# FrancescoI/torchrecsys

Measured on AMD Instinct MI355X. Metric: training interactions/sec (pos+neg), higher is better.
Workload: dtype f32; 1 GPU; c4 per-GPU shard: net_type='fm', 10M users x 1M items, 125M-interaction shard of 1B, dim=128, per-GPU batch 32768 (global 262144 at 8 GPUs); global_batch=32768, per_gpu_batch=32768, rng=device (Feistel epoch shuffle + Philox4x32-10 negative sampler)

## Files before the change

### torchrecsys_amd/csrc/api.cpp

```cpp
#include "trs_common.h"

#include <string.h>

static thread_local char g_err[512] = "";

void trs_set_error(const char* fmt, ...) {
  va_list ap;
  va_start(ap, fmt);
  vsnprintf(g_err, sizeof(g_err), fmt, ap);
  va_end(ap);
}

extern "C" const char* trs_last_error(void) { return g_err; }

#include <mutex>
#include <stdlib.h>

namespace {
struct Knob {
  const char* name;
  int64_t TrsTuning::*wide;
  int TrsTuning::*narrow;
  int64_t unset;
};
const Knob KNOBS[] = {
    {"GRID_CAP", &TrsTuning::grid_cap, nullptr, 256 * 16},
    {"PASS_GRID_CAP", &TrsTuning::pass_grid_cap, nullptr, 4096},
    {"PRESORT_GRID_CAP", &TrsTuning::presort_grid_cap, nullptr, 512},
    {"K1_ITERS", nullptr, &TrsTuning::k1_iters, 0},
    {"PASS_ITERS", nullptr, &TrsTuning::pass_iters, 0},
    {"PASS_NT", nullptr, &TrsTuning::pass_nt, -1},
    {"K1_NT", nullptr, &TrsTuning::k1_nt, -1},
    {"K1_WGS_PER_CU", nullptr, &TrsTuning::k1_wgs_per_cu, 2},
    {"K1_APPLY_IN_LOOP", nullptr, &TrsTuning::k1_apply_in_loop, 1},
    {"K1_APPLY_STATS", nullptr, &TrsTuning::k1_apply_stats, 0},
    {"GEMM32_NO_GLDS", nullptr, &TrsTuning::gemm32_no_glds, 0},
    {"GEMM16_TN_WIDE", nullptr, &TrsTuning::gemm16_tn_wide, -1},
    {"GEMM16_TILE", nullptr, &TrsTuning::gemm16_tile, 0},
    {"GEMM16_NO_GLDS", nullptr, &TrsTuning::gemm16_no_glds, 0},
    {"BN_FINAL_TWO_SWEEPS", nullptr, &TrsTuning::bn_final_two_sweeps, 0},
    {"FOLDIN_DEPTH", nullptr, &TrsTuning::foldin_depth, 4},
    {"RANKS_STAGES", nullptr, &TrsTuning::ranks_stages, 3},
    {"EASE_STAGES", nullptr, &TrsTuning::ease_stages, 7},
};
TrsTuning g_tuning;
std::once_flag g_tuning_once;
void knob_store(const Knob& k, int64_t v) {
  if (k.wide) g_tuning.*(k.wide) = v;
  else g_tuning.*(k.narrow) = (int)v;
}
}

TrsTuning& trs_tuning() {
  std::call_once(g_tuning_once, [] {
    for (const Knob& k : KNOBS) {
      char name[64];
      snprintf(name, sizeof(name), "TRS_%s", k.name);
      const char* e = getenv(name);
      knob_store(k, (e && *e) ? atoll(e) : k.unset);
    }
  });
  return g_tuning;
}

extern "C" int trs_tuning_set(const char* name, int64_t value, int32_t unset) {
  TRS_REQUIRE(name != nullptr, "trs_tuning_set: NULL name");
  (void)trs_tuning();
  for (const Knob& k : KNOBS)
    if (strcmp(k.name, name) == 0) {
      knob_store(k, unset ? k.unset : value);
      return TRS_OK;
    }
  trs_set_error("trs_tuning_set: unknown knob %s", name);
  return TRS_E_ARG;
}

extern "C" int trs_abi_version(void) { return TRS_ABI_VERSION; }

extern "C" int trs_check_device(void) {
  int dev = -1;
  if (hipGetDevice(&dev) != hipSuccess) {
    trs_set_error("trs_check_device: no HIP device");
    (void)hipGetLastError();
    return TRS_E_DEVICE;
  }
  hipDeviceProp_t p;
  if (hipGetDeviceProperties(&p, dev) != hipSuccess) {
    trs_set_error("trs_check_device: hipGetDeviceProperties failed");
    (void)hipGetLastError();
    return TRS_E_DEVICE;
  }
  if (strncmp(p.gcnArchName, "gfx950", 6) != 0) {
    trs_set_error("trs_check_device: device %d is %s, this library is built for gfx950 only", dev, p.gcnArchName);
    return TRS_E_DEVICE;
  }
  return TRS_OK;
}

extern "C" int trs_events_create(int32_t n, void** handles_out) {
  TRS_REQUIRE(n >= 0 && (n == 0 || handles_out), "trs_events_create: bad arguments");
  for (int32_t i = 0; i < n; ++i) {
    hipEvent_t e;
    if (hipEventCreate(&e) != hipSuccess) {
      trs_set_error("trs_events_create: hipEventCreate failed");
      (void)hipGetLastError();
      return TRS_E_LAUNCH;
    }
    handles_out[i] = (void*)e;
  }
  return TRS_OK;
}

extern "C" int trs_events_destroy(int32_t n, void** handles) {
  for (int32_t i = 0; i < n; ++i)
    if (handles && handles[i]) (void)hipEventDestroy((hipEvent_t)handles[i]);
  return TRS_OK;
}

// ... 10 lines not shown
```

### torchrecsys_amd/csrc/fast_step.hip

```cpp
#include "score_kernels.h"
#include "opt_rows.h"

#include <math.h>
#include <stdlib.h>

namespace trs {

struct FastArgs {
  trs_tables T;
  int32_t* user;
  int32_t* pos;
  int32_t* neg;
  int64_t B;
  int32_t* err;
  int from_stream;
  const int2* sui;
  const int32_t* neg_static;
  int64_t N;
  uint64_t shuffle_key;
  int hb;
  int64_t t0;
  uint64_t sample_seed;
  uint64_t sample_offset;
  float* gz;
  float* du;
  float inv_B;
  float lr;
  int loss;
  float* loss_sum;
  uint64_t* uown;
  uint64_t* iown;
  uint32_t* udup;
  uint32_t* idup;
  uint32_t stamp;
  const uint8_t* udup_pos;
  const uint8_t* idup_pos;
  float* ustage;
  OptArgs o;
  uint32_t* sync;
  uint32_t sync_base, sync_target;
  const int32_t* nflag;
  int apply_in_loop, apply_stats;
};

struct RawIds {
  int32_t u, p, n;
  uint8_t dup;
  uint16_t idup;
  int64_t v;
  bool valid;
};

struct TripleIds {
  int32_t u, p, n;
  bool valid, ok, dup, pdup, ndup;
};

template <int SRC, int INL>
__device__ __forceinline__ RawIds issue_ids(const FastArgs& a, int64_t t) {
  RawIds r;
  r.valid = t < a.B;
  const int64_t tc = r.valid ? t : a.B - 1;
  r.v = 0;
  if (SRC != 0) {
    const int64_t p = trs_feistel_perm(a.t0 + tc, a.N, a.shuffle_key, a.hb);
    const int2 ui = a.sui[p];
    r.u = ui.x;
    r.p = ui.y;
    if (SRC == 2) {
      r.n = a.neg_static[p];
    } else {
      const trs_u4 x = trs_philox4x32_10(a.sample_offset + (uint64_t)tc, a.sample_seed);
      const uint64_t x64 = ((uint64_t)x.y << 32) | (uint64_t)x.x;
      r.v = a.T.n_items > 1 ? (int64_t)trs_mulhi64(x64, (uint64_t)(a.T.n_items - 1)) : 0;
      r.n = 0;
    }
  } else {
    r.u = a.user[tc];
    r.p = a.pos[tc];
    r.n = a.neg[tc];
  }
  r.dup = 1;
  r.idup = 0x0101;
  if (INL) r.dup = a.udup_pos[tc];
  if (INL >= 2) r.idup = reinterpret_cast<const uint16_t*>(a.idup_pos)[tc];
  return r;
}

template <int SRC>
__device__ __forceinline__ TripleIds finalize_ids(const FastArgs& a, const RawIds& w) {
  TripleIds r;
  r.valid = w.valid;
  int64_t uid = w.u, pid = w.p;
  int64_t nid = SRC == 1 ? (a.T.n_items > 1 ? w.v + (w.v >= pid ? 1 : 0) : 0) : (int64_t)w.n;
  r.ok = true;
  if ((uint64_t)uid >= (uint64_t)a.T.n_users) { r.ok = false; uid = 0; }
  if ((uint64_t)pid >= (uint64_t)a.T.n_items) { r.ok = false; pid = 0; }
  if ((uint64_t)nid >= (uint64_t)a.T.n_items) { r.ok = false; nid = 0; }
  r.u = (int32_t)uid;
  r.p = (int32_t)pid;
  r.n = (int32_t)nid;
  r.dup = w.dup != 0;
  r.pdup = (w.idup & 0x00ffu) != 0;
  r.ndup = (w.idup & 0xff00u) != 0;
  return r;
}

template <int VEC, int K>
struct TripleRows {
  RowReg<VEC, K> u, pi, ni;
  float ul, pl, nl;
  RowReg<VEC, K> us1, us2;
  float uls1, uls2;
};

template <int VEC, int G, int K, bool FULL, int OPT, int NTU = 0>
__device__ __forceinline__ void load_rows(TripleRows<VEC, K>& r, const trs_tables& T, const OptArgs& o,
                                          const TripleIds& id, int lig) {
  row_load<VEC, G, K, FULL, (NTU & 1) != 0>(r.u, T.user, id.u, T.D, lig);
  row_load<VEC, G, K, FULL>(r.pi, T.item, id.p, T.D, lig);
  row_load<VEC, G, K, FULL>(r.ni, T.item, id.n, T.D, lig);
  r.ul = T.user_lin[id.u];
  r.pl = T.item_lin[id.p];
  r.nl = T.item_lin[id.n];
  if (OPT != OPT_SGD) {
    row_load<VEC, G, K, FULL>(r.us1, o.user_s1, id.u, T.D, lig);
    r.uls1 = o.user_lin_s1[id.u];
    if (OPT == OPT_ADAM) {
      row_load<VEC, G, K, FULL>(r.us2, o.user_s2, id.u, T.D, lig);
      r.uls2 = o.user_lin_s2[id.u];
    }
  }
}

constexpr int DEFER_ITERS = 8;
struct DeferEntry {
  uint32_t tw;
  int32_t row;
  float c;
  float clin;
};

template <int NET, int VEC, int G, int K, int SRC, bool FULL, int INL, int OPT = OPT_SGD, int NTU = 0>
__global__ __launch_bounds__(TRS_BLOCK, (INL == 3 && VEC == 4 && G >= 4 && K == 1 && FULL) ? 4 : 1) void fwd_stage_kernel(const FastArgs a) {
  constexpr int N = K * VEC;
  constexpr int TPW = TRS_WAVE / G;
  constexpr bool DEFER = INL == 3;
  constexpr int NWV = TRS_BLOCK / TRS_WAVE;
  constexpr int LIST_CAP = DEFER ? NWV * DEFER_ITERS * TPW * 3 : 1;
  __shared__ DeferEntry s_list[LIST_CAP];
  __shared__ int s_total;
  const trs_tables& T = a.T;
  const int D = T.D;
  const int64_t B = a.B;
  const int lane = threadIdx.x & 63;
  const int lig = lane % G;
  const int64_t wave = ((int64_t)blockIdx.x * TRS_BLOCK + threadIdx.x) >> 6;
  const int64_t nwave = ((int64_t)gridDim.x * TRS_BLOCK) >> 6;
  const int64_t stride = nwave * TPW;
  float loss_acc = 0.f;

#ifdef TRS_K1_STAMPS
  uint64_t* stamps = reinterpret_cast<uint64_t*>(a.gz) + 8 * (int64_t)blockIdx.x;
  if (INL == 3 && threadIdx.x == 0) {
    stamps[0] = __builtin_amdgcn_s_memrealtime();
    stamps[4] = 0;
  }
#endif
  __shared__ int s_arr;
  __shared__ int s_left;
  int64_t fi = 0;
  bool early = false, arrived = false;
  if (DEFER) {
    if (threadIdx.x == 0) s_total = s_arr = s_left = 0;
    if (a.nflag) {
      const int64_t nf = *a.nflag;
      fi = (nf + stride - 1) / stride;
      early = fi < (B + stride - 1) / stride;
    }
    __syncthreads();
  }
  auto arrive = [&]() {
    int before = 0;
    if (lane == 0) before = atomicAdd(&s_arr, 1);
    before = __builtin_amdgcn_readfirstlane(before);
    if (before == NWV - 1 && lane == 0)
      (void)__hip_atomic_fetch_add(a.sync, 1u, __ATOMIC_RELAXED, __HIP_MEMORY_SCOPE_AGENT);
    arrived = true;
  };
  constexpr int CAPW = DEFER_ITERS * TPW * 3, DU = 4, KDD = (N * G + TRS_WAVE - 1) / TRS_WAVE;
  const int wv = __builtin_amdgcn_readfirstlane((int)(threadIdx.x >> 6));
  int my_cnt = 0, next_e = 0;
  bool complete = false;
  auto entry_at = [&](int e) -> int { return early ? wv * CAPW + e : wv + NWV * e; };
  auto load_round = [&](float (&x)[DU][KDD], int e0, int n_mine) {
#pragma unroll
    for (int k = 0; k < DU; ++k) {
      const bool has = e0 + k < n_mine;
      const DeferEntry en = s_list[has ? entry_at(e0 + k) : 0];
      const int64_t tk = has ? (int64_t)(en.tw >> 2) : 0;
      const float* src = ((en.tw & 3u) == 0 ? a.du : a.ustage) + tk * (int64_t)D;
#pragma unroll
      for (int q = 0; q < KDD; ++q) {
        const int e = q * TRS_WAVE + lane;
        x[k][q] = __hip_atomic_load(src + (e < D ? e : 0), __ATOMIC_RELAXED, __HIP_MEMORY_SCOPE_AGENT);
      }
    }
  };
  auto apply_round = [&](float (&x)[DU][KDD], int e0, int n_mine) {
#pragma unroll
    for (int k = 0; k < DU; ++k) {
      if (e0 + k >= n_mine) continue;
      const DeferEntry en = s_list[entry_at(e0 + k)];
      const int which = (int)(en.tw & 3u);
      float* dst = (which == 0 ? T.user : T.item) + (int64_t)en.row * D;
#pragma unroll
      for (int q = 0; q < KDD; ++q) {
        const int e = q * TRS_WAVE + lane;
        if (e < D) atomicAdd(dst + e, en.c * x[k][q]);
      }
      if (lane == 0) atomicAdd((which == 0 ? T.user_lin : T.item_lin) + en.row, en.clin);
    }
  };
  int64_t t = wave * TPW + lane / G;
// ... 1018 lines not shown
static int launch_meta_stage_mt(const ScoreArgs& a, hipStream_t s) {
  RowCfg c;
  TRS_TRY(row_cfg_for("launch_meta_stage", a.T.D, c));
  const int tpw = TRS_WAVE / c.g;
  int64_t iters = (a.Bt.B + 512 * 4 * (int64_t)tpw - 1) / (512 * 4 * (int64_t)tpw);
  iters = iters < 2 ? 2 : (iters > 8 ? 8 : iters);
  int64_t grid = ((a.Bt.B + tpw - 1) / tpw + 4 * iters - 1) / (4 * iters);
  grid = grid < 1 ? 1 : (grid > 4096 ? 4096 : grid);
  const dim3 gr((unsigned)grid), bl(TRS_BLOCK);
  return for_whole_row_shape(c, [&](auto V, auto G, auto K) {
    const bool full = V() * G() * K() == a.T.D;
    if (a.o.kind != OPT_SGD) {
      if (!full) return 1;
      if (a.o.kind == OPT_ADAM)
        hipLaunchKernelGGL((meta_stage_kernel<NET, V(), G(), K(), true, MT, OPT_ADAM>), gr, bl, 0, s, a);
      else
        hipLaunchKernelGGL((meta_stage_kernel<NET, V(), G(), K(), true, MT, OPT_ADAGRAD>), gr, bl, 0, s, a);
    } else if (full)
      hipLaunchKernelGGL((meta_stage_kernel<NET, V(), G(), K(), true, MT>), gr, bl, 0, s, a);
    else
      hipLaunchKernelGGL((meta_stage_kernel<NET, V(), G(), K(), false, MT>), gr, bl, 0, s, a);
    TRS_CHECK_LAUNCH("meta_stage_kernel");
    return TRS_OK;
  });
}

template <int NET>
static int launch_meta_stage(const ScoreArgs& a, hipStream_t s) {
  if (!a.Bt.pos_meta || !a.Bt.neg_meta || a.grad_rows) return 1;
  switch (a.T.M) {
    case 1: return launch_meta_stage_mt<NET, 1>(a, s);
    case 2: return launch_meta_stage_mt<NET, 2>(a, s);
    case 3: return launch_meta_stage_mt<NET, 3>(a, s);
    default: return 1;
  }
}

template <typename KernelT>
static int64_t defer_resident_cap(KernelT kernel) {
  int occ = 0, dev = 0, cus = 0;
  if (hipOccupancyMaxActiveBlocksPerMultiprocessor(&occ, kernel, TRS_BLOCK, 0) != hipSuccess) return 0;
  if (hipGetDevice(&dev) != hipSuccess ||
      hipDeviceGetAttribute(&cus, hipDeviceAttributeMultiprocessorCount, dev) != hipSuccess)
    return 0;
  const int want = trs_tuning().k1_wgs_per_cu;
  const int per_cu = occ - 1 < want ? occ - 1 : want;
  return per_cu > 0 ? (int64_t)per_cu * cus : 0;
}

enum StepForm { STEP_MARKS, STEP_SORTED_MARKS, STEP_SORTED, STEP_FLAGS };
struct StepPlan {
  StepForm form;
  int src;
  int inl;
  int item_bits;
  bool owners;
  bool adaptive;
  bool user_pairs;
  bool meta;
  bool meta_ids;
  bool meta_sorted;
  bool sync;
  bool nflag;
};

template <int NET>
static int launch_fwd_stage(const FastArgs& a, const StepPlan& p, hipStream_t s, uint32_t* deferred) {
  *deferred = 0;
  RowCfg c;
  TRS_TRY(row_cfg_for("launch_fwd_stage", a.T.D, c));
  const int tpw = TRS_WAVE / c.g;
  const int iters_env = trs_tuning().k1_iters;
  int64_t iters = iters_env > 0 ? iters_env : (a.B + 512 * 4 * (int64_t)tpw - 1) / (512 * 4 * (int64_t)tpw);
  if (iters < 2) iters = 2;
  if (iters > 8 && iters_env <= 0) iters = 8;
  int64_t grid = ((a.B + tpw - 1) / tpw + 4 * iters - 1) / (4 * iters);
  if (grid < 1) grid = 1;
  if (grid > 4096) grid = 4096;
  const int ntu_env = trs_tuning().k1_nt;
  const int ntu = ntu_env >= 0 ? ntu_env : ((int64_t)a.T.n_users * a.T.D * 4 > ((int64_t)512 << 20) ? 3 : 0);
  const dim3 gr((unsigned)grid), bl(TRS_BLOCK);
  return for_row_shape(c, [&](auto V, auto G, auto K) {
    constexpr int VV = V(), GG = G(), KK = K();
    auto launch = [&](auto FULL) {
      constexpr bool FU = FULL();
      if (p.inl == 1 && a.o.kind == OPT_ADAM)
        hipLaunchKernelGGL((fwd_stage_kernel<NET, VV, GG, KK, 0, FU, 1, OPT_ADAM>), gr, bl, 0, s, a);
      else if (p.inl == 1 && a.o.kind == OPT_ADAGRAD)
        hipLaunchKernelGGL((fwd_stage_kernel<NET, VV, GG, KK, 0, FU, 1, OPT_ADAGRAD>), gr, bl, 0, s, a);
      else if (p.inl == 1)
        hipLaunchKernelGGL((fwd_stage_kernel<NET, VV, GG, KK, 0, FU, 1>), gr, bl, 0, s, a);
      else if (p.inl == 3 && iters <= DEFER_ITERS) {
        static const int64_t cap = defer_resident_cap(fwd_stage_kernel<NET, VV, GG, KK, 0, FU, 3>);
        if (grid <= cap) {
          FastArgs b = a;
          b.sync_target = a.sync_base + (uint32_t)grid;
          b.apply_in_loop = trs_tuning().k1_apply_in_loop != 0;
          b.apply_stats = trs_tuning().k1_apply_stats != 0;
          if (ntu == 1)
            hipLaunchKernelGGL((fwd_stage_kernel<NET, VV, GG, KK, 0, FU, 3, OPT_SGD, 1>), gr, bl, 0, s, b);
          else if (ntu == 3)
            hipLaunchKernelGGL((fwd_stage_kernel<NET, VV, GG, KK, 0, FU, 3, OPT_SGD, 3>), gr, bl, 0, s, b);
          else
            hipLaunchKernelGGL((fwd_stage_kernel<NET, VV, GG, KK, 0, FU, 3>), gr, bl, 0, s, b);
          *deferred = (uint32_t)grid;
        } else
          hipLaunchKernelGGL((fwd_stage_kernel<NET, VV, GG, KK, 0, FU, 2>), gr, bl, 0, s, a);
      } else if (p.inl >= 2)
        hipLaunchKernelGGL((fwd_stage_kernel<NET, VV, GG, KK, 0, FU, 2>), gr, bl, 0, s, a);
      else if (p.src == 0) hipLaunchKernelGGL((fwd_stage_kernel<NET, VV, GG, KK, 0, FU, 0>), gr, bl, 0, s, a);
      else if (p.src == 1) hipLaunchKernelGGL((fwd_stage_kernel<NET, VV, GG, KK, 1, FU, 0>), gr, bl, 0, s, a);
      else hipLaunchKernelGGL((fwd_stage_kernel<NET, VV, GG, KK, 2, FU, 0>), gr, bl, 0, s, a);
    };
    if (VV * GG * KK == a.T.D) launch(std::true_type{});
    else launch(std::false_type{});
    TRS_CHECK_LAUNCH("fwd_stage_kernel");
    return TRS_OK;
  });
}

static int launch_flagged_update(const FastArgs& a, hipStream_t s) {
  const dim3 gr(trs_grid((3 * a.B + FLG_REFS - 1) / FLG_REFS, TRS_BLOCK / TRS_WAVE)), bl(TRS_BLOCK);
  const int kd = (a.T.D + TRS_WAVE - 1) / TRS_WAVE;
  if (kd <= 1) hipLaunchKernelGGL(flagged_update_kernel<1>, gr, bl, 0, s, a);
  else if (kd <= 2) hipLaunchKernelGGL(flagged_update_kernel<2>, gr, bl, 0, s, a);
  else if (kd <= 4) hipLaunchKernelGGL(flagged_update_kernel<4>, gr, bl, 0, s, a);
  else if (kd <= 8) hipLaunchKernelGGL(flagged_update_kernel<8>, gr, bl, 0, s, a);
  else hipLaunchKernelGGL(flagged_update_kernel<16>, gr, bl, 0, s, a);
  TRS_CHECK_LAUNCH("flagged_update_kernel");
  return TRS_OK;
}

template <int WHICH>
static int launch_plain(const FastArgs& a, hipStream_t s) {
  RowCfg c;
  TRS_TRY(row_cfg_for("launch_plain", a.T.D, c));
  const int per = (TRS_WAVE / c.g) * 2;
  const dim3 gr(trs_grid((a.B + per - 1) / per, TRS_BLOCK / TRS_WAVE)), bl(TRS_BLOCK);
  return for_row_shape(c, [&](auto V, auto G, auto K) {
    constexpr int VV = V(), GG = G(), KK = K();
    auto launch = [&](auto FULL) {
      if (WHICH == 0) hipLaunchKernelGGL((item_owner_update_kernel<VV, GG, KK, FULL()>), gr, bl, 0, s, a);
      else if (WHICH == 1) hipLaunchKernelGGL((user_plain_update_kernel<VV, GG, KK, FULL()>), gr, bl, 0, s, a);
      else hipLaunchKernelGGL((user_dup_update_kernel<VV, GG, KK, FULL()>), gr, bl, 0, s, a);
    };
    if (VV * GG * KK == a.T.D) launch(std::true_type{});
    else launch(std::false_type{});
    TRS_CHECK_LAUNCH("plain update kernel");
    return TRS_OK;
  });
}

static int launch_updates(const FastArgs& a, bool owners, hipStream_t s, hipEvent_t ev_k3) {
  const int D = a.T.D;
  if (owners) {
    int rc = launch_plain<0>(a, s);
    if (rc) return rc;
  }
#define TRS_UPD(L, KD, U)                                                                            \
  {                                                                                                  \
    constexpr int PER = (TRS_WAVE / L) * U;                                                          \
    const dim3 gr(trs_grid((a.B + PER - 1) / PER, TRS_BLOCK / TRS_WAVE)), bl(TRS_BLOCK);             \
    if (owners) {                                                                                    \
      hipLaunchKernelGGL((item_update_kernel<L, KD, U, 2>), gr, bl, 0, s, a);                        \
      if (ev_k3) (void)hipEventRecord(ev_k3, s);                                                     \
    } else {                                                                                         \
// ... 411 lines not shown
```

### torchrecsys_amd/csrc/trs_common.h

```cpp
#pragma once
#include <hip/hip_runtime.h>
#include <stdint.h>
#include <stdio.h>
#include <stdarg.h>
#include <stdlib.h>

#include "../../include/trs.h"

#define TRS_WAVE 64
#define TRS_BLOCK 256

void trs_set_error(const char* fmt, ...);

#define TRS_REQUIRE(cond, ...)        \
  do {                                \
    if (!(cond)) {                    \
      trs_set_error(__VA_ARGS__);     \
      return TRS_E_ARG;               \
    }                                 \
  } while (0)

#define TRS_TRY(expr)           \
  do {                          \
    const int rc__ = (expr);    \
    if (rc__) return rc__;      \
  } while (0)

#define TRS_CHECK_LAUNCH(name)                                           \
  do {                                                                     \
    hipError_t e__ = hipGetLastError();                                    \
    if (e__ != hipSuccess) {                                               \
      trs_set_error("%s: launch failed: %s", name, hipGetErrorString(e__)); \
      return TRS_E_LAUNCH;                                                 \
    }                                                                      \
  } while (0)

static inline double trs_as_written(float x) {
  char buf[40];
  for (int digits = 1; digits <= 9; ++digits) {
    snprintf(buf, sizeof buf, "%.*g", digits, (double)x);
    if (strtof(buf, nullptr) == x) return strtod(buf, nullptr);
  }
  return (double)x;
}

struct TrsTuning {
  int64_t grid_cap;
  int64_t pass_grid_cap;
  int64_t presort_grid_cap;
  int k1_iters;
  int pass_iters;
  int pass_nt;
  int k1_nt;
  int k1_wgs_per_cu;
  int k1_apply_in_loop;
  int k1_apply_stats;
  int gemm32_no_glds;
  int gemm16_tn_wide;
  int gemm16_tile;
  int gemm16_no_glds;
  int bn_final_two_sweeps;
  int foldin_depth;
  int ranks_stages;
  int ease_stages;
};
TrsTuning& trs_tuning();

static inline int trs_grid(int64_t work_items, int items_per_block) {
  const int64_t cap = trs_tuning().grid_cap;
  int64_t g = (work_items + items_per_block - 1) / items_per_block;
  if (g < 1) g = 1;
  if (g > cap) g = cap;
  return (int)g;
}

__device__ __forceinline__ int64_t trs_ld_idx(const void* p, int idx_bytes, int64_t t) {
  return idx_bytes == 8 ? ((const int64_t*)p)[t] : (int64_t)((const int32_t*)p)[t];
}
__device__ __forceinline__ void trs_st_idx(void* p, int idx_bytes, int64_t t, int64_t v) {
  if (idx_bytes == 8)
    ((int64_t*)p)[t] = v;
  else
    ((int32_t*)p)[t] = (int32_t)v;
}

struct trs_u4 {
  uint32_t x, y, z, w;
};
__host__ __device__ __forceinline__ trs_u4 trs_philox4x32_10(uint64_t counter, uint64_t key) {
  uint32_t c0 = (uint32_t)counter, c1 = (uint32_t)(counter >> 32), c2 = 0u, c3 = 0u;
  uint32_t k0 = (uint32_t)key, k1 = (uint32_t)(key >> 32);
#pragma unroll
  for (int r = 0; r < 10; ++r) {
    uint64_t p0 = (uint64_t)0xD2511F53u * c0;
    uint64_t p1 = (uint64_t)0xCD9E8D57u * c2;
    uint32_t n0 = (uint32_t)(p1 >> 32) ^ c1 ^ k0;
    uint32_t n1 = (uint32_t)p1;
    uint32_t n2 = (uint32_t)(p0 >> 32) ^ c3 ^ k1;
    uint32_t n3 = (uint32_t)p0;
    c0 = n0; c1 = n1; c2 = n2; c3 = n3;
    k0 += 0x9E3779B9u;
    k1 += 0xBB67AE85u;
  }
  trs_u4 o = {c0, c1, c2, c3};
  return o;
}

__host__ __device__ __forceinline__ uint64_t trs_mulhi64(uint64_t a, uint64_t b) {
#ifdef __HIP_DEVICE_COMPILE__
  return __umul64hi(a, b);
#else
  return (uint64_t)(((unsigned __int128)a * (unsigned __int128)b) >> 64);
#endif
}

__host__ __device__ __forceinline__ int64_t trs_sample_one_neg(uint64_t seed, uint64_t ctr, int64_t pos,
                                                               int64_t n_items) {
  trs_u4 r = trs_philox4x32_10(ctr, seed);
  uint64_t x = ((uint64_t)r.y << 32) | (uint64_t)r.x;
  if (n_items <= 1) return 0;
  int64_t v = (int64_t)trs_mulhi64(x, (uint64_t)(n_items - 1));
  return v + (v >= pos ? 1 : 0);
}

__device__ __forceinline__ void trs_pair_loss(int kind, float sp, float sn, float& value, float& dneg) {
  if (kind == TRS_LOSS_BPR) {
    const float x = sn - sp;
    value = fmaxf(x, 0.f) + log1pf(expf(-fabsf(x)));
    dneg = 1.0f / (1.0f + expf(-x));
  } else {
    const float h = sn - sp + 1.0f;
    value = fmaxf(h, 0.f);
    dneg = h >= 0.f ? 1.f : 0.f;
  }
}

struct TrsSampler {
  int k_neg, popularity, max_tries;
  const int64_t* seen_off;
// ... 168 lines not shown
```

Measured before the change: 2.106 billion interactions/s.

## Add specialized flag-step kernel for deferred in-kernel duplicate apply path

Adds a new flag_step_kernel, in its own translation unit, for the INL==3 deferred-apply path when a whole row fits one row shape. It keeps the first iteration's user rows and gradients in registers so held duplicate updates can be applied from registers via LDS rather than reloaded from global staging buffers. It also pipelines applies into the tail loop once the grid-wide sync counter is complete. The kernel is enabled by default through a new K1_FLAG_KERNEL knob, gated on B <= 49152 and on a resident-grid cap, and falls back to the old kernel otherwise. The aim is fewer global round-trips and an earlier apply phase, at the cost of more register and LDS pressure and a separately compiled kernel.

```diff
diff --git a/torchrecsys_amd/csrc/api.cpp b/torchrecsys_amd/csrc/api.cpp
--- a/torchrecsys_amd/csrc/api.cpp
+++ b/torchrecsys_amd/csrc/api.cpp
@@ -34,6 +34,7 @@
     {"K1_WGS_PER_CU", nullptr, &TrsTuning::k1_wgs_per_cu, 2},
     {"K1_APPLY_IN_LOOP", nullptr, &TrsTuning::k1_apply_in_loop, 1},
     {"K1_APPLY_STATS", nullptr, &TrsTuning::k1_apply_stats, 0},
+    {"K1_FLAG_KERNEL", nullptr, &TrsTuning::k1_flag_kernel, 1},
     {"GEMM32_NO_GLDS", nullptr, &TrsTuning::gemm32_no_glds, 0},
     {"GEMM16_TN_WIDE", nullptr, &TrsTuning::gemm16_tn_wide, -1},
     {"GEMM16_TILE", nullptr, &TrsTuning::gemm16_tile, 0},
diff --git a/torchrecsys_amd/csrc/fast_step.hip b/torchrecsys_amd/csrc/fast_step.hip
--- a/torchrecsys_amd/csrc/fast_step.hip
+++ b/torchrecsys_amd/csrc/fast_step.hip
@@ -1,145 +1,7 @@
-#include "score_kernels.h"
-#include "opt_rows.h"
-
-#include <math.h>
-#include <stdlib.h>
+#include "fast_step_args.h"
 
 namespace trs {
 
-struct FastArgs {
-  trs_tables T;
-  int32_t* user;
-  int32_t* pos;
-  int32_t* neg;
-  int64_t B;
-  int32_t* err;
-  int from_stream;
-  const int2* sui;
-  const int32_t* neg_static;
-  int64_t N;
-  uint64_t shuffle_key;
-  int hb;
-  int64_t t0;
-  uint64_t sample_seed;
-  uint64_t sample_offset;
-  float* gz;
-  float* du;
-  float inv_B;
-  float lr;
-  int loss;
-  float* loss_sum;
-  uint64_t* uown;
-  uint64_t* iown;
-  uint32_t* udup;
-  uint32_t* idup;
-  uint32_t stamp;
-  const uint8_t* udup_pos;
-  const uint8_t* idup_pos;
-  float* ustage;
-  OptArgs o;
-  uint32_t* sync;
-  uint32_t sync_base, sync_target;
-  const int32_t* nflag;
-  int apply_in_loop, apply_stats;
-};
-
-struct RawIds {
-  int32_t u, p, n;
-  uint8_t dup;
-  uint16_t idup;
-  int64_t v;
-  bool valid;
-};
-
-struct TripleIds {
-  int32_t u, p, n;
-  bool valid, ok, dup, pdup, ndup;
-};
-
-template <int SRC, int INL>
-__device__ __forceinline__ RawIds issue_ids(const FastArgs& a, int64_t t) {
-  RawIds r;
-  r.valid = t < a.B;
-  const int64_t tc = r.valid ? t : a.B - 1;
-  r.v = 0;
-  if (SRC != 0) {
-    const int64_t p = trs_feistel_perm(a.t0 + tc, a.N, a.shuffle_key, a.hb);
-    const int2 ui = a.sui[p];
-    r.u = ui.x;
-    r.p = ui.y;
-    if (SRC == 2) {
-      r.n = a.neg_static[p];
-    } else {
-      const trs_u4 x = trs_philox4x32_10(a.sample_offset + (uint64_t)tc, a.sample_seed);
-      const uint64_t x64 = ((uint64_t)x.y << 32) | (uint64_t)x.x;
-      r.v = a.T.n_items > 1 ? (int64_t)trs_mulhi64(x64, (uint64_t)(a.T.n_items - 1)) : 0;
-      r.n = 0;
-    }
-  } else {
-    r.u = a.user[tc];
-    r.p = a.pos[tc];
-    r.n = a.neg[tc];
-  }
-  r.dup = 1;
-  r.idup = 0x0101;
-  if (INL) r.dup = a.udup_pos[tc];
-  if (INL >= 2) r.idup = reinterpret_cast<const uint16_t*>(a.idup_pos)[tc];
-  return r;
-}
-
-template <int SRC>
-__device__ __forceinline__ TripleIds finalize_ids(const FastArgs& a, const RawIds& w) {
-  TripleIds r;
-  r.valid = w.valid;
-  int64_t uid = w.u, pid = w.p;
-  int64_t nid = SRC == 1 ? (a.T.n_items > 1 ? w.v + (w.v >= pid ? 1 : 0) : 0) : (int64_t)w.n;
-  r.ok = true;
-  if ((uint64_t)uid >= (uint64_t)a.T.n_users) { r.ok = false; uid = 0; }
-  if ((uint64_t)pid >= (uint64_t)a.T.n_items) { r.ok = false; pid = 0; }
-  if ((uint64_t)nid >= (uint64_t)a.T.n_items) { r.ok = false; nid = 0; }
-  r.u = (int32_t)uid;
-  r.p = (int32_t)pid;
-  r.n = (int32_t)nid;
-  r.dup = w.dup != 0;
-  r.pdup = (w.idup & 0x00ffu) != 0;
-  r.ndup = (w.idup & 0xff00u) != 0;
-  return r;
-}
-
-template <int VEC, int K>
-struct TripleRows {
-  RowReg<VEC, K> u, pi, ni;
-  float ul, pl, nl;
-  RowReg<VEC, K> us1, us2;
-  float uls1, uls2;
-};
-
-template <int VEC, int G, int K, bool FULL, int OPT, int NTU = 0>
-__device__ __forceinline__ void load_rows(TripleRows<VEC, K>& r, const trs_tables& T, const OptArgs& o,
-                                          const TripleIds& id, int lig) {
-  row_load<VEC, G, K, FULL, (NTU & 1) != 0>(r.u, T.user, id.u, T.D, lig);
-  row_load<VEC, G, K, FULL>(r.pi, T.item, id.p, T.D, lig);
-  row_load<VEC, G, K, FULL>(r.ni, T.item, id.n, T.D, lig);
-  r.ul = T.user_lin[id.u];
-  r.pl = T.item_lin[id.p];
-  r.nl = T.item_lin[id.n];
-  if (OPT != OPT_SGD) {
-    row_load<VEC, G, K, FULL>(r.us1, o.user_s1, id.u, T.D, lig);
-    r.uls1 = o.user_lin_s1[id.u];
-    if (OPT == OPT_ADAM) {
-      row_load<VEC, G, K, FULL>(r.us2, o.user_s2, id.u, T.D, lig);
-      r.uls2 = o.user_lin_s2[id.u];
-    }
-  }
-}
-
-constexpr int DEFER_ITERS = 8;
-struct DeferEntry {
-  uint32_t tw;
-  int32_t row;
-  float c;
-  float clin;
-};
 
 template <int NET, int VEC, int G, int K, int SRC, bool FULL, int INL, int OPT = OPT_SGD, int NTU = 0>
 __global__ __launch_bounds__(TRS_BLOCK, (INL == 3 && VEC == 4 && G >= 4 && K == 1 && FULL) ? 4 : 1) void fwd_stage_kernel(const FastArgs a) {
@@ -1324,6 +1186,11 @@
   const dim3 gr((unsigned)grid), bl(TRS_BLOCK);
   return for_row_shape(c, [&](auto V, auto G, auto K) {
     constexpr int VV = V(), GG = G(), KK = K();
+    if (p.inl == 3 && p.sync && p.nflag && iters <= DEFER_ITERS && VV * GG * KK == a.T.D) {
+      const int rc = trs_launch_flag_step(NET, a, c, ntu, grid, s);
+      if (rc == TRS_OK) *deferred = (uint32_t)grid;
+      if (rc <= 0) return rc;
+    }
     auto launch = [&](auto FULL) {
       constexpr bool FU = FULL();
       if (p.inl == 1 && a.o.kind == OPT_ADAM)
diff --git a/torchrecsys_amd/csrc/fast_step_args.h b/torchrecsys_amd/csrc/fast_step_args.h
--- /dev/null
+++ b/torchrecsys_amd/csrc/fast_step_args.h
@@ -0,0 +1,147 @@
+#pragma once
+#include "score_kernels.h"
+#include "opt_rows.h"
+
+#include <math.h>
+#include <stdlib.h>
+
+namespace trs {
+
+struct FastArgs {
+  trs_tables T;
+  int32_t* user;
+  int32_t* pos;
+  int32_t* neg;
+  int64_t B;
+  int32_t* err;
+  int from_stream;
+  const int2* sui;
+  const int32_t* neg_static;
+  int64_t N;
+  uint64_t shuffle_key;
+  int hb;
+  int64_t t0;
+  uint64_t sample_seed;
+  uint64_t sample_offset;
+  float* gz;
+  float* du;
+  float inv_B;
+  float lr;
+  int loss;
+  float* loss_sum;
+  uint64_t* uown;
+  uint64_t* iown;
+  uint32_t* udup;
+  uint32_t* idup;
+  uint32_t stamp;
+  const uint8_t* udup_pos;
+  const uint8_t* idup_pos;
+  float* ustage;
+  OptArgs o;
+  uint32_t* sync;
+  uint32_t sync_base, sync_target;
+  const int32_t* nflag;
+  int apply_in_loop, apply_stats;
+};
+
+struct RawIds {
+  int32_t u, p, n;
+  uint8_t dup;
+  uint16_t idup;
+  int64_t v;
+  bool valid;
+};
+
+struct TripleIds {
+  int32_t u, p, n;
+  bool valid, ok, dup, pdup, ndup;
+};
+
+template <int SRC, int INL>
+__device__ __forceinline__ RawIds issue_ids(const FastArgs& a, int64_t t) {
+  RawIds r;
+  r.valid = t < a.B;
+  const int64_t tc = r.valid ? t : a.B - 1;
+  r.v = 0;
+  if (SRC != 0) {
+    const int64_t p = trs_feistel_perm(a.t0 + tc, a.N, a.shuffle_key, a.hb);
+    const int2 ui = a.sui[p];
+    r.u = ui.x;
+    r.p = ui.y;
+    if (SRC == 2) {
+      r.n = a.neg_static[p];
+    } else {
+      const trs_u4 x = trs_philox4x32_10(a.sample_offset + (uint64_t)tc, a.sample_seed);
+      const uint64_t x64 = ((uint64_t)x.y << 32) | (uint64_t)x.x;
+      r.v = a.T.n_items > 1 ? (int64_t)trs_mulhi64(x64, (uint64_t)(a.T.n_items - 1)) : 0;
+      r.n = 0;
+    }
+  } else {
+    r.u = a.user[tc];
+    r.p = a.pos[tc];
+    r.n = a.neg[tc];
+  }
+  r.dup = 1;
+  r.idup = 0x0101;
+  if (INL) r.dup = a.udup_pos[tc];
+  if (INL >= 2) r.idup = reinterpret_cast<const uint16_t*>(a.idup_pos)[tc];
+  return r;
+}
+
+template <int SRC>
+__device__ __forceinline__ TripleIds finalize_ids(const FastArgs& a, const RawIds& w) {
+  TripleIds r;
+  r.valid = w.valid;
+  int64_t uid = w.u, pid = w.p;
+  int64_t nid = SRC == 1 ? (a.T.n_items > 1 ? w.v + (w.v >= pid ? 1 : 0) : 0) : (int64_t)w.n;
+  r.ok = true;
+  if ((uint64_t)uid >= (uint64_t)a.T.n_users) { r.ok = false; uid = 0; }
+  if ((uint64_t)pid >= (uint64_t)a.T.n_items) { r.ok = false; pid = 0; }
+  if ((uint64_t)nid >= (uint64_t)a.T.n_items) { r.ok = false; nid = 0; }
+  r.u = (int32_t)uid;
+  r.p = (int32_t)pid;
+  r.n = (int32_t)nid;
+  r.dup = w.dup != 0;
+  r.pdup = (w.idup & 0x00ffu) != 0;
+  r.ndup = (w.idup & 0xff00u) != 0;
+  return r;
+}
+
+template <int VEC, int K>
+struct TripleRows {
+  RowReg<VEC, K> u, pi, ni;
+  float ul, pl, nl;
+  RowReg<VEC, K> us1, us2;
+  float uls1, uls2;
+};
+
+template <int VEC, int G, int K, bool FULL, int OPT, int NTU = 0>
+__device__ __forceinline__ void load_rows(TripleRows<VEC, K>& r, const trs_tables& T, const OptArgs& o,
+                                          const TripleIds& id, int lig) {
+  row_load<VEC, G, K, FULL, (NTU & 1) != 0>(r.u, T.user, id.u, T.D, lig);
+  row_load<VEC, G, K, FULL>(r.pi, T.item, id.p, T.D, lig);
+  row_load<VEC, G, K, FULL>(r.ni, T.item, id.n, T.D, lig);
+  r.ul = T.user_lin[id.u];
+  r.pl = T.item_lin[id.p];
+  r.nl = T.item_lin[id.n];
+  if (OPT != OPT_SGD) {
+    row_load<VEC, G, K, FULL>(r.us1, o.user_s1, id.u, T.D, lig);
+    r.uls1 = o.user_lin_s1[id.u];
+    if (OPT == OPT_ADAM) {
+      row_load<VEC, G, K, FULL>(r.us2, o.user_s2, id.u, T.D, lig);
+      r.uls2 = o.user_lin_s2[id.u];
+    }
+  }
+}
+
+constexpr int DEFER_ITERS = 8;
+struct DeferEntry {
+  uint32_t tw;
+  int32_t row;
+  float c;
+  float clin;
+};
+
+int trs_launch_flag_step(int net, const FastArgs& a, const RowCfg& c, int ntu, int64_t grid, void* stream);
+
+}
diff --git a/torchrecsys_amd/csrc/flag_step.hip b/torchrecsys_amd/csrc/flag_step.hip
--- /dev/null
+++ b/torchrecsys_amd/csrc/flag_step.hip
@@ -0,0 +1,373 @@
+#include "fast_step_args.h"
+
+namespace trs {
+
+#ifndef TRS_FLAG_STEP_ORDER
+#define TRS_FLAG_STEP_ORDER 0
+#endif
+
+template <int NET, int G, int NTU>
+__global__ __launch_bounds__(TRS_BLOCK, 3) void flag_step_kernel(const FastArgs a) {
+  constexpr int VEC = 4, K = 1, N = 4, D = 4 * G;
+  constexpr int TPW = TRS_WAVE / G;
+  constexpr int NWV = TRS_BLOCK / TRS_WAVE;
+  constexpr int CAPW = DEFER_ITERS * TPW * 3, DU = 4, KDD = (D + TRS_WAVE - 1) / TRS_WAVE;
+  constexpr int FLAG_APPLY = KDD >= 4 ? 1 : 2;
+  __shared__ DeferEntry s_list[NWV * CAPW];
+  __shared__ float s_turn[NWV * D];
+  __shared__ float s_loss[NWV];
+  __shared__ int s_arr;
+  __shared__ int s_left;
+  const trs_tables& T = a.T;
+  const int64_t B = a.B;
+  const int lane = threadIdx.x & 63;
+  const int lig = lane % G;
+  const int grp = lane / G;
+  const int wv = __builtin_amdgcn_readfirstlane((int)(threadIdx.x >> 6));
+  const int64_t wave = ((int64_t)blockIdx.x * TRS_BLOCK + threadIdx.x) >> 6;
+  const int64_t nwave = ((int64_t)gridDim.x * TRS_BLOCK) >> 6;
+  const int64_t stride = nwave * TPW;
+  float loss_acc = 0.f;
+
+  if (threadIdx.x == 0) s_arr = s_left = 0;
+  const int64_t fi = ((int64_t)*a.nflag + stride - 1) / stride;
+  __syncthreads();
+  bool arrived = false;
+  auto arrive = [&](float pin) __attribute__((always_inline)) {
+    asm volatile("" ::"v"(pin) : "memory");
+    int before = 0;
+    if (lane == 0) before = atomicAdd(&s_arr, 1);
+    before = __builtin_amdgcn_readfirstlane(before);
+    if (before == NWV - 1 && lane == 0)
+      (void)__hip_atomic_fetch_add(a.sync, 1u, TRS_FLAG_STEP_ORDER >= 1 ? __ATOMIC_RELEASE : __ATOMIC_RELAXED,
+                                   __HIP_MEMORY_SCOPE_AGENT);
+    arrived = true;
+  };
+
+  RowReg<VEC, K> hU0, hU1, hG0, hG1;
+#pragma unroll
+  for (int n = 0; n < N; ++n) hU0.v[n] = hU1.v[n] = hG0.v[n] = hG1.v[n] = 0.f;
+  int my_cnt = 0, n_held = 0, next_e = 0;
+  bool complete = false;
+
+  auto apply_held = [&](int e) __attribute__((always_inline)) {
+    const DeferEntry ev = s_list[wv * CAPW + e];
+    const uint32_t tw = (uint32_t)__builtin_amdgcn_readfirstlane((int)ev.tw);
+    const int row = __builtin_amdgcn_readfirstlane(ev.row);
+    const float c = __int_as_float(__builtin_amdgcn_readfirstlane(__float_as_int(ev.c)));
+    const float clin = __int_as_float(__builtin_amdgcn_readfirstlane(__float_as_int(ev.clin)));
+    const int which = (int)(tw & 3u);
+    const bool s1 = (tw & 8u) != 0;
+    const int eg = (int)(tw >> 4);
+    float hv[N];
+#pragma unroll
+    for (int n = 0; n < N; ++n) {
+      const float g0 = hG0.v[n], g1 = hG1.v[n], u0 = hU0.v[n], u1 = hU1.v[n];
+      const float gs = s1 ? g1 : g0, us = s1 ? u1 : u0;
+      hv[n] = which == 0 ? gs : us;
+    }
+    const float4 h = make_float4(hv[0], hv[1], hv[2], hv[3]);
+    float* turn = s_turn + wv * D;
+    asm volatile("" ::: "memory");
+    if (grp == eg) *reinterpret_cast<float4*>(turn + 4 * lig) = h;
+    asm volatile("" ::: "memory");
+    float x[KDD];
+#pragma unroll
+    for (int q = 0; q < KDD; ++q) {
+      const int el = q * TRS_WAVE + lane;
+      x[q] = turn[el < D ? el : 0];
+    }
+    asm volatile("" ::: "memory");
+    float* dst = (which == 0 ? T.user : T.item) + (int64_t)row * D;
+#pragma unroll
+    for (int q = 0; q < KDD; ++q) {
+      const int el = q * TRS_WAVE + lane;
+      if (el < D) atomicAdd(dst + el, c * x[q]);
+    }
+    if (lane == 0) atomicAdd((which == 0 ? T.user_lin : T.item_lin) + row, clin);
+  };
+  auto load_round = [&](float (&x)[DU][KDD], int e0, int n_mine) {
+#pragma unroll
+    for (int k = 0; k < DU; ++k) {
+      const bool has = e0 + k < n_mine;
+      const DeferEntry en = s_list[wv * CAPW + (has ? e0 + k : 0)];
+      const int64_t tk = has ? (int64_t)(en.tw >> 3) : 0;
+      const float* src = ((en.tw & 3u) == 0 ? a.du : a.ustage) + tk * (int64_t)D;
+#pragma unroll
+      for (int q = 0; q < KDD; ++q) {
+        const int el = q * TRS_WAVE + lane;
+        x[k][q] = __hip_atomic_load(src + (el < D ? el : 0), __ATOMIC_RELAXED, __HIP_MEMORY_SCOPE_AGENT);
+      }
+    }
+  };
+  auto apply_round = [&](float (&x)[DU][KDD], int e0, int n_mine) {
+#pragma unroll
+    for (int k = 0; k < DU; ++k) {
+      if (e0 + k >= n_mine) continue;
+      const DeferEntry en = s_list[wv * CAPW + e0 + k];
+      const int which = (int)(en.tw & 3u);
+      float* dst = (which == 0 ? T.user : T.item) + (int64_t)en.row * D;
+#pragma unroll
+      for (int q = 0; q < KDD; ++q) {
+        const int el = q * TRS_WAVE + lane;
+        if (el < D) atomicAdd(dst + el, en.c * x[k][q]);
+      }
+      if (lane == 0) atomicAdd((which == 0 ? T.user_lin : T.item_lin) + en.row, en.clin);
+    }
+  };
+  auto apply_rest = [&](int from) __attribute__((always_inline)) {
+#pragma nounroll
+    for (int e = from; e < n_held; ++e) apply_held(e);
+    float x[DU][KDD];
+    for (int e0 = from > n_held ? from : n_held; e0 < my_cnt; e0 += DU) {
+      load_round(x, e0, my_cnt);
+      apply_round(x, e0, my_cnt);
+    }
+  };
+
+  int64_t t = wave * TPW + grp;
+  const int64_t t_first = wave * TPW;
+  const int64_t niter = t_first < B ? (B - t_first + stride - 1) / stride : 0;
+  const int nph = __builtin_amdgcn_readfirstlane((int)((niter + 1) & ~(int64_t)1));
+  const int ia = nph - 3;
+  const bool inloop = __builtin_amdgcn_readfirstlane(a.apply_in_loop != 0 && ia >= 1 && fi < (int64_t)ia) != 0;
+  uint32_t seen_l = 0;
+  int n_loop = 0;
+  auto look = [&](int ph) __attribute__((always_inline)) {
+    if (inloop && ph == ia && __builtin_amdgcn_readfirstlane(n_held) > 0) {
+      seen_l = __hip_atomic_load(a.sync, __ATOMIC_RELAXED, __HIP_MEMORY_SCOPE_AGENT);
+      n_loop = __builtin_amdgcn_readfirstlane(n_held);
+    }
+  };
+  auto consume = [&](int ph) __attribute__((always_inline)) {
+    if (n_loop > next_e && ph >= ia) {
+      if (ph == ia) {
+        complete = (int32_t)((uint32_t)__builtin_amdgcn_readfirstlane((int)seen_l) - a.sync_target) >= 0;
+        if (TRS_FLAG_STEP_ORDER >= 2 && complete) __builtin_amdgcn_fence(__ATOMIC_ACQUIRE, "agent");
+      }
+      if (complete) {
+#pragma nounroll
+        for (int k = 0; k < FLAG_APPLY && next_e < n_loop; ++k) apply_held(next_e++);
+      }
+    }
+  };
+
+  auto reduce = [&](TripleRows<VEC, K>& r, const TripleIds& id, int64_t tt, auto SLOT, bool hold) __attribute__((always_inline)) -> float {
+    const bool live = id.valid && id.ok;
+    if (id.valid && !id.ok && lig == 0 && a.err) atomicOr(a.err, 1);
+    float pp = 0.f, pn = 0.f;
+    if (NET == TRS_NET_FM) {
+#pragma unroll
+      for (int n = 0; n < N; ++n) {
+        const float sp_ = r.u.v[n] + r.pi.v[n], sn_ = r.u.v[n] + r.ni.v[n];
+        const float uu = r.u.v[n] * r.u.v[n];
+        pp += sp_ * sp_ - (uu + r.pi.v[n] * r.pi.v[n]);
+        pn += sn_ * sn_ - (uu + r.ni.v[n] * r.ni.v[n]);
+      }
+    } else {
+#pragma unroll
+      for (int n = 0; n < N; ++n) {
+        pp += r.u.v[n] * r.pi.v[n];
+        pn += r.u.v[n] * r.ni.v[n];
+      }
+    }
+    pp = trs_group_sum<G>(pp);
+    pn = trs_group_sum<G>(pn);
+    float sp, sn;
+    if (NET == TRS_NET_FM) {
+      sp = sigmoidf_((r.ul + r.pl) + 0.5f * pp);
+      sn = sigmoidf_((r.ul + r.nl) + 0.5f * pn);
+    } else {
+      sp = (pp + r.ul) + r.pl;
+      sn = (pn + r.ul) + r.nl;
+    }
+    float lval, dneg;
+    trs_pair_loss(a.loss, sp, sn, lval, dneg);
+    const float act = live ? dneg : 0.f;
+    float gp = -act * a.inv_B, gn = act * a.inv_B;
+    if (live && lig == 0) loss_acc += lval;
+    if (NET == TRS_NET_FM) {
+      gp = gp * ((1.0f - sp) * sp);
+      gn = gn * ((1.0f - sn) * sn);
+    }
+    RowReg<VEC, K> g;
+#pragma unroll
+    for (int n = 0; n < N; ++n) g.v[n] = gp * r.pi.v[n] + gn * r.ni.v[n];
+    {
+      const bool lead = lig == 0 && live;
+      const uint64_t mu = __ballot(lead && id.dup), mp = __ballot(lead && id.pdup), mn = __ballot(lead && id.ndup);
+      const uint64_t below = ((uint64_t)1 << lane) - 1;
+      const int cu = __popcll(mu), cp = __popcll(mp), cn = __popcll(mn);
+      const int bu = wv * CAPW + my_cnt;
+      my_cnt += cu + cp + cn;
+      if (arrived && (cu + cp + cn) && lane == 0 && a.err) atomicOr(a.err, 8);
+      constexpr int slot = decltype(SLOT)::value;
+      const uint32_t tw = hold ? (4u | ((uint32_t)slot << 3) | ((uint32_t)grp << 4)) : ((uint32_t)tt << 3);
+      const int bp = bu + cu, bn = bp + cp;
+      if (lead && id.dup) s_list[bu + __popcll(mu & below)] = {tw, id.u, -a.lr, -a.lr * (gp + gn)};
+      if (lead && id.pdup) s_list[bp + __popcll(mp & below)] = {tw | 1u, id.p, -a.lr * gp, -a.lr * gp};
+      if (lead && id.ndup) s_list[bn + __popcll(mn & below)] = {tw | 2u, id.n, -a.lr * gn, -a.lr * gn};
+    }
+    if (hold) {
+      if constexpr (decltype(SLOT)::value == 0) {
+        hU0 = r.u;
+        hG0 = g;
+      } else {
+        hU1 = r.u;
+        hG1 = g;
+      }
+    }
+    if (id.valid) {
+      if (!hold && (id.pdup || id.ndup)) row_store<VEC, G, K>(r.u, a.ustage + tt * (int64_t)D, D, lig);
+      if (live) {
+        const float cp = -a.lr * gp, cn = -a.lr * gn;
+        if (!id.pdup) {
+          RowReg<VEC, K> o;
+#pragma unroll
+          for (int n = 0; n < N; ++n) o.v[n] = r.pi.v[n] + cp * r.u.v[n];
+          row_store<VEC, G, K>(o, T.item + id.p * (int64_t)D, D, lig);
+          if (lig == 0) T.item_lin[id.p] = r.pl + cp;
+        }
+        if (!id.ndup) {
+          RowReg<VEC, K> o;
+#pragma unroll
+          for (int n = 0; n < N; ++n) o.v[n] = r.ni.v[n] + cn * r.u.v[n];
+          row_store<VEC, G, K>(o, T.item + id.n * (int64_t)D, D, lig);
+          if (lig == 0) T.item_lin[id.n] = r.nl + cn;
+        }
+      }
+      if (id.dup || !live) {
+        if (!hold) row_store<VEC, G, K>(g, a.du + tt * (int64_t)D, D, lig);
+      } else {
+        RowReg<VEC, K> un;
+#pragma unroll
+        for (int n = 0; n < N; ++n) un.v[n] = r.u.v[n] + (-a.lr) * g.v[n];
+        row_store<VEC, G, K, (NTU & 2) != 0>(un, T.user + id.u * (int64_t)D, D, lig);
+        if (lig == 0) T.user_lin[id.u] = r.ul + (-a.lr) * (gp + gn);
+      }
+    }
+    return gp + gn;
+  };
+
+  TripleIds idE, idO;
+  TripleRows<VEC, K> rE, rO;
+  {
+    constexpr std::integral_constant<int, 0> S0{};
+    constexpr std::integral_constant<int, 1> S1{};
+    RawIds wE = issue_ids<0, 3>(a, t);
+    RawIds wO = issue_ids<0, 3>(a, t + stride);
+    idE = finalize_ids<0>(a, wE);
+    load_rows<VEC, G, K, true, OPT_SGD, NTU>(rE, T, a.o, idE, lig);
+    if (fi == 0) arrive(0.f);
+    for (int it = 0; it < nph; it += 2) {
+      const bool first = it == 0;
+      wE = issue_ids<0, 3>(a, t + 2 * stride);
+      idO = finalize_ids<0>(a, wO);
+      load_rows<VEC, G, K, true, OPT_SGD, NTU>(rO, T, a.o, idO, lig);
+      const float pe = reduce(rE, idE, t, S0, first);
+      if (first) n_held = my_cnt;
+      if ((int64_t)it + 1 == fi) arrive(pe);
+      consume(it);
+      look(it + 1);
+
+      wO = issue_ids<0, 3>(a, t + 3 * stride);
+      idE = finalize_ids<0>(a, wE);
+      load_rows<VEC, G, K, true, OPT_SGD, NTU>(rE, T, a.o, idE, lig);
+      const float po = reduce(rO, idO, t + stride, S1, first);
+      if (first) n_held = my_cnt;
+      if ((int64_t)it + 2 == fi) arrive(po);
+      consume(it + 1);
+      t += 2 * stride;
+    }
+    if (!arrived) arrive(loss_acc);
+  }
+  const float wl = trs_wave_sum(loss_acc);
+  if (lane == 0) s_loss[wv] = wl;
+  const int n_in_loop = next_e;
+  if (my_cnt > next_e) {
+    const uint32_t seen = __hip_atomic_load(a.sync, __ATOMIC_RELAXED, __HIP_MEMORY_SCOPE_AGENT);
+    asm volatile("s_waitcnt vmcnt(0)" ::: "memory");
+    complete = (int32_t)((uint32_t)__builtin_amdgcn_readfirstlane((int)seen) - a.sync_target) >= 0;
+    if (complete) {
+      if (TRS_FLAG_STEP_ORDER >= 2) __builtin_amdgcn_fence(__ATOMIC_ACQUIRE, "agent");
+      apply_rest(next_e);
+      next_e = my_cnt;
+    } else if (lane == 0) {
+      s_left = 1;
+    }
+  }
+  asm volatile("s_waitcnt vmcnt(0)" ::: "memory");
+  __syncthreads();
+  if (threadIdx.x == 0) {
+    float L = 0.f;
+#pragma unroll
+    for (int w = 0; w < NWV; ++w) L += s_loss[w];
+    if (L != 0.f) atomicAdd(a.loss_sum, L);
+  }
+  if (a.apply_stats && lane == 0) {
+    uint32_t* st = a.sync + (TRS_SYNC_WORDS - 2);
+    if (n_in_loop) (void)__hip_atomic_fetch_add(st, (uint32_t)n_in_loop, __ATOMIC_RELAXED, __HIP_MEMORY_SCOPE_AGENT);
+    if (my_cnt > n_in_loop)
+      (void)__hip_atomic_fetch_add(st + 1, (uint32_t)(my_cnt - n_in_loop), __ATOMIC_RELAXED, __HIP_MEMORY_SCOPE_AGENT);
+  }
+  if (!s_left) return;
+  if (threadIdx.x == 0) {
+    const uint64_t t_start = __builtin_amdgcn_s_memrealtime();
+    const uint64_t limit = (a.err && (__hip_atomic_load(a.err, __ATOMIC_RELAXED, __HIP_MEMORY_SCOPE_AGENT) & 4)) ? 0ull : 5000000ull;
+    while ((int32_t)(__hip_atomic_load(a.sync, __ATOMIC_RELAXED, __HIP_MEMORY_SCOPE_AGENT) - a.sync_target) < 0) {
+      __builtin_amdgcn_s_sleep(6);
+      if (__builtin_amdgcn_s_memrealtime() - t_start > limit) {
+        if (a.err) atomicOr(a.err, 4);
+        break;
+      }
+    }
+  }
+  __syncthreads();
+  if (TRS_FLAG_STEP_ORDER >= 2) __builtin_amdgcn_fence(__ATOMIC_ACQUIRE, "agent");
+  apply_rest(next_e);
+}
+
+template <typename KernelT>
+static int64_t flag_resident_cap(KernelT kernel) {
+  int occ = 0, dev = 0, cus = 0;
+  if (hipOccupancyMaxActiveBlocksPerMultiprocessor(&occ, kernel, TRS_BLOCK, 0) != hipSuccess) return 0;
+  if (hipGetDevice(&dev) != hipSuccess ||
+      hipDeviceGetAttribute(&cus, hipDeviceAttributeMultiprocessorCount, dev) != hipSuccess)
+    return 0;
+  const int want = trs_tuning().k1_wgs_per_cu;
+  const int per_cu = occ - 1 < want ? occ - 1 : want;
+  return per_cu > 0 ? (int64_t)per_cu * cus : 0;
+}
+
+template <int NET>
+static int launch_flag_step(const FastArgs& a, const RowCfg& c, int ntu, int64_t grid, hipStream_t s) {
+  const dim3 gr((unsigned)grid), bl(TRS_BLOCK);
+  return for_whole_row_shape(c, [&](auto V, auto G, auto K) {
+    constexpr int GG = G();
+    if (V() * GG * K() != a.T.D) return 1;
+    static const int64_t cap = flag_resident_cap(flag_step_kernel<NET, GG, 0>);
+    if (grid > cap) return 1;
+    FastArgs b = a;
+    b.sync_target = a.sync_base + (uint32_t)grid;
+    b.apply_in_loop = trs_tuning().k1_apply_in_loop != 0;
+    b.apply_stats = trs_tuning().k1_apply_stats != 0;
+    if (ntu == 1) hipLaunchKernelGGL((flag_step_kernel<NET, GG, 1>), gr, bl, 0, s, b);
+    else if (ntu == 3) hipLaunchKernelGGL((flag_step_kernel<NET, GG, 3>), gr, bl, 0, s, b);
+    else hipLaunchKernelGGL((flag_step_kernel<NET, GG, 0>), gr, bl, 0, s, b);
+    TRS_CHECK_LAUNCH("flag_step_kernel");
+    return TRS_OK;
+  });
+}
+
+int trs_launch_flag_step(int net, const FastArgs& a, const RowCfg& c, int ntu, int64_t grid, void* stream) {
+#ifdef TRS_K1_STAMPS
+  return 1;
+#endif
+  if (trs_tuning().k1_flag_kernel == 0 || !a.nflag || !a.sync) return 1;
+  if (a.B > 4 * 12288) return 1;
+  hipStream_t s = (hipStream_t)stream;
+  return net == TRS_NET_FM ? launch_flag_step<TRS_NET_FM>(a, c, ntu, grid, s)
+                           : launch_flag_step<TRS_NET_LINEAR>(a, c, ntu, grid, s);
+}
+
+}
diff --git a/torchrecsys_amd/csrc/trs_common.h b/torchrecsys_amd/csrc/trs_common.h
--- a/torchrecsys_amd/csrc/trs_common.h
+++ b/torchrecsys_amd/csrc/trs_common.h
@@ -55,6 +55,7 @@
   int k1_wgs_per_cu;
   int k1_apply_in_loop;
   int k1_apply_stats;
+  int k1_flag_kernel;
   int gemm32_no_glds;
   int gemm16_tn_wide;
   int gemm16_tile;
```

Result: faster. 2.153 billion interactions/s (median of 6 runs) (+2.2%).
